# mutiann/few-shot-transformer-tts

Hardware: AMD Instinct MI355X
Metric: padded mel-frames/sec, full training step (fwd+loss+bwd+allreduce+Adam) (higher is better)
Workload: dtype bf16; 1 GPU; LJSpeech-shaped (BASELINE configs[1]) packed batch per GPU: B=14 S=114 T=582, default hparams (83.5M params), dropout on, single speaker/language; global_batch=14, seq_len=582, parallelism=dp1

## Files before the change

few-shot-transformer-tts_amd/csrc/capi_ops.hip:

```cpp
#include "engine.h"
#include "attention.h"
#include "enc_fused.h"

namespace {
inline hipStream_t S_(void* s) { return (hipStream_t)s; }
inline int rup8(int x) { return (x + 7) & ~7; }
__global__ void k_dropmask(DropCfg d, uint8_t* out, long n) {
    long i = (long)blockIdx.x * blockDim.x + threadIdx.x;
    if (i < n) out[i] = b2s_keep(d, (uint32_t)i) ? 1 : 0;
}
}

int b2s_attn_core_fwd_export(int dtype, hipStream_t st, const void* q, int ldq, const void* k, int ldk, const void* v, int ldv,
                             void* ctx, int ldc, int B, int H, int Lq, int Lk, int dh, int mask_mode, const int* klen,
                             const float* bias, long bias_sb, long bias_sq, DropCfg drop, float* S, void* P, void* Pd);
int b2s_attn_core_bwd_export(int dtype, hipStream_t st, const void* dctx, int ldc, const void* q, int ldq, const void* k, int ldk,
                             const void* v, int ldv, const void* P, const void* Pd, void* dq, int lddq, void* dk, int lddk,
                             void* dv, int lddv, int B, int H, int Lq, int Lk, int dh, DropCfg drop, float* dP, void* dS);

extern "C" int b2s_gemm(const b2s_gemm_desc* d, const void* A, const void* B, void* C, const float* bias,
                        const float* residual, const int32_t* row_len, const int32_t* conv_len, void* stream) {
    B2S_CHECK(d && A && B && C, "null argument");
    GemmArgs g;
    g.M = d->M; g.N = d->N; g.K = d->K; g.batch = d->batch > 0 ? d->batch : 1; g.batch_inner = d->batch_inner > 0 ? d->batch_inner : 1;
    g.A.p = A; g.A.ld = d->lda; g.A.bs_o = d->a_bs_o; g.A.bs_i = d->a_bs_i;
    g.B.p = B; g.B.ld = d->ldb; g.B.bs_o = d->b_bs_o; g.B.bs_i = d->b_bs_i;
    if (d->trans_a) { g.A.R = d->K; g.A.C = d->M; } else { g.A.R = d->M; g.A.C = d->K; }
    if (d->trans_b) { g.B.R = d->K; g.B.C = d->N; } else { g.B.R = d->N; g.B.C = d->K; }
    if (d->conv_cin_a > 0) {
        B2S_CHECK(!d->trans_a, "conv gather is defined on the row-major A operand");
        g.A.g_cin = d->conv_cin_a; g.A.g_T = d->conv_T; g.A.g_len = conv_len; g.A.R = d->M; g.A.C = d->K;
    }
    g.C = C; g.c_fp32 = d->c_fp32; g.ldc = d->ldc; g.cs_o = d->c_bs_o; g.cs_i = d->c_bs_i;
    g.epi.alpha = d->alpha; g.epi.bias = bias; g.epi.relu = d->relu; g.epi.accumulate = d->accumulate;
    g.epi.drop = make_drop(d->drop_p, d->seed, 7u);
    g.epi.residual = residual; g.epi.ldr = d->ldc;
    g.epi.row_len = row_len; g.epi.rows_per_batch = d->rows_per_batch > 0 ? d->rows_per_batch : 1;
    g.epi.conv_dw_cin = d->conv_dw_cin;
    return b2s_gemm_launch(g, d->dtype, d->trans_a != 0, d->trans_b != 0, S_(stream));
}
extern "C" int b2s_gemm_splitk(const b2s_gemm_desc* d, int splitk, const void* A, const void* B, float* C, float* ws, size_t ws_floats,
                               void* stream) {
    B2S_CHECK(d && A && B && C && splitk >= 1, "null argument / bad split");
    B2S_CHECK(d->c_fp32 && d->accumulate && !d->relu && d->drop_p == 0.f && d->conv_cin_a == 0, "split-K needs a linear fp32 accumulate epilogue");
    GemmArgs g;
    g.M = d->M; g.N = d->N; g.K = d->K; g.batch = d->batch > 0 ? d->batch : 1; g.batch_inner = d->batch_inner > 0 ? d->batch_inner : 1;
    g.A.p = A; g.A.ld = d->lda; g.A.bs_o = d->a_bs_o; g.A.bs_i = d->a_bs_i;
    g.B.p = B; g.B.ld = d->ldb; g.B.bs_o = d->b_bs_o; g.B.bs_i = d->b_bs_i;
    if (d->trans_a) { g.A.R = d->K; g.A.C = d->M; } else { g.A.R = d->M; g.A.C = d->K; }
    if (d->trans_b) { g.B.R = d->K; g.B.C = d->N; } else { g.B.R = d->N; g.B.C = d->K; }
    g.C = C; g.c_fp32 = 1; g.ldc = d->ldc; g.cs_o = d->c_bs_o; g.cs_i = d->c_bs_i;
    g.epi.alpha = d->alpha; g.epi.accumulate = 1; g.epi.conv_dw_cin = d->conv_dw_cin;
    g.splitk = splitk; g.ws = ws; g.ws_floats = ws ? ws_floats : 0;
// ... 151 lines not shown
```

few-shot-transformer-tts_amd/csrc/engine.hip:

```cpp
#include <algorithm>
#include <cmath>
#include <cstdarg>
#include <cstdlib>
#include "engine.h"
#include "attention.h"
#include "enc_fused.h"
#include "drop_sites.h"

thread_local char g_b2s_err[512] = "";
int b2s_fail(const char* file, int line, const char* fmt, ...) {
    char msg[400];
    va_list ap; va_start(ap, fmt); vsnprintf(msg, sizeof(msg), fmt, ap); va_end(ap);
    const char* base = strrchr(file, '/');
    snprintf(g_b2s_err, sizeof(g_b2s_err), "%s:%d: %s", base ? base + 1 : file, line, msg);
    return 1;
}

int b2s_model::id(const std::string& n) const {
    auto it = index.find(n);
    return it == index.end() ? -1 : it->second;
}

namespace {

// ... 571 lines not shown
    const int rings = m->dw_group ? cf.n_decoder_layer : 1;
    for (int i = 0; i < (rings == 1 ? 1 : 3 * rings); ++i) sc.r_dyT.push_back(a.T(M * D, esz));
    for (int i = 0; i < (rings == 1 ? 1 : 2 * rings); ++i) sc.r_dqkv.push_back(a.T(M * 3 * D, esz));
    for (int i = 0; i < rings; ++i) { sc.r_dz.push_back(a.T(M * 4 * D, esz)); sc.r_dkv.push_back(a.T(Mk * 2 * D, esz)); }
    sc.dyT = sc.r_dyT[0]; sc.dz = sc.r_dz[0]; sc.dqkv = sc.r_dqkv[0]; sc.dkv = sc.r_dkv[0];
    sc.dctx = a.T(M * D, esz); sc.dh = a.T(M * D, esz); sc.dx = a.f32(M * D);
    sc.dmelT = a.T(M * cf.num_mels, esz); sc.doutT = a.T(M * D, esz); sc.da3 = a.T(M * D, esz);
    sc.dz1 = a.T(M * cf.prenet_hidden, esz); sc.dz2 = a.T(M * cf.prenet_hidden, esz);
    sc.dstop_m = a.f32(M);
    if (m->kv_cat) sc.dkvcat = a.T(Mk * cf.n_decoder_layer * 2 * D, esz);
    sc.lnws = a.f32((long)RO_LN_WS_ROWS * 2 * D);
    for (int i = 0; i < (m->dw_group ? 3 * cf.n_decoder_layer + 2 : RO_LN_BATCH); ++i) sc.r_lnws.push_back(a.f32((long)RO_LN_WS_ROWS * 2 * D));
    if (m->kv_cat) { sc.dctx_x = a.T(M * D, esz); sc.dsum_x = a.f32((long)B * H * T); }
}

struct PostScratch { std::vector<void*> du, dy; float* stat; int stat_stride; void* col = nullptr; };
void plan_postnet(const b2s_model* m, b2s_ctx& c, Arena& a, PostScratch& ps) {
    const b2s_config& cf = m->cfg;
    const long M = (long)c.B * c.T;
    const int n = cf.n_postnet_layer, esz = m->esz;
    c.u.assign(n, nullptr); c.y.assign(n, nullptr); c.bn_mean.assign(n, nullptr); c.bn_rstd.assign(n, nullptr);
    ps.du.assign(n + 1, nullptr);
    for (int i = 0; i < n; ++i) {
        int cin = i == 0 ? cf.num_mels : cf.postnet_hidden;
        int cout = i == n - 1 ? cf.num_mels : cf.postnet_hidden;
        c.u[i] = a.T(M * cin, esz);
        c.y[i] = a.f32(M * cout);
        c.bn_mean[i] = a.f32(cout); c.bn_rstd[i] = a.f32(cout);
        ps.du[i] = a.T(M * cin, esz);
    }
    int maxc = std::max(cf.num_mels, cf.postnet_hidden);
    ps.du[n] = a.T(M * maxc, esz);
    ps.dy.assign(n, nullptr);
    for (int i = 0; i < n; ++i) ps.dy[i] = a.T(M * (i == n - 1 ? cf.num_mels : cf.postnet_hidden), esz);
    ps.stat_stride = 2 * maxc;
    ps.stat = a.f32((long)n * ps.stat_stride);
    if (m->dtype == 1) ps.col = a.T(M * 5 * maxc, esz);
}

int check_bound(const b2s_model* m) {
    B2S_CHECK(m && m->bound, "model parameters are not bound (call b2s_model_bind first)");
    return 0;
}

}

extern "C" const char* b2s_last_error(void) { return g_b2s_err; }
extern "C" int b2s_version(void) { return 100; }

extern "C" int b2s_model_create(const b2s_config* cfg, b2s_model** out) {
    B2S_CHECK(cfg && out, "null argument");
    const b2s_config& c = *cfg;
// ... 1184 lines not shown
}

extern "C" int b2s_postnet_backward(b2s_model* m, b2s_ctx* c, const float* d_out, float* d_inputs_out, int flags, void* stream) {
    B2S_TRY(check_bound(m));
    B2S_CHECK(c && c->kind == 3 && d_out && d_inputs_out, "bad postnet context");
    B2S_CHECK(c->train, "postnet backward requires a train-mode forward (batch statistics)");
    const b2s_config& cf = m->cfg;
    hipStream_t st = S_(stream);
    const int B = c->B, T = c->T, n = cf.n_postnet_layer, dt = m->dtype;
    const long M = (long)B * T;
    const float pd = cf.decoder_dropout_rate;
    Arena a; a.base = c->ws; a.cap = c->ws_bytes;
    b2s_ctx tmp; tmp.B = B; tmp.T = T;
    PostScratch ps;
    plan_postnet(m, tmp, a, ps);
    std::vector<GemmArgs> dws;
    for (int i = n - 1; i >= 0; --i) {
        const int cin = i == 0 ? cf.num_mels : cf.postnet_hidden, cout = i == n - 1 ? cf.num_mels : cf.postnet_hidden;
        const std::string q = "postnet.batchnorm_layers." + std::to_string(i) + ".";
        DropCfg d = make_drop(pd, c->seed, drop_op(DS_POST_CONV, i));
        const void* dout = i == n - 1 ? (const void*)d_out : ps.du[i + 1];
        void* dy = ps.dy[i];
        B2S_TRY(ro_bn_bwd(dt, dout, i == n - 1 ? 1 : 0, c->y[i], c->bn_mean[i], c->bn_rstd[i], m->P(q + "weight"), m->P(q + "bias"),
                          i < n - 1 ? 1 : 0, m->G(q + "weight"), m->G(q + "bias"), dy, (int)M, cout, d, st));
        {
            GemmArgs g;
            g.A.p = dy; g.A.ld = cout; g.A.R = (int)M; g.A.C = cout;
            g.B.p = c->u[i]; g.B.ld = cin; g.B.R = (int)M; g.B.C = 5 * cin; g.B.g_cin = cin; g.B.g_T = T; g.B.g_len = c->tgt_len;
            g.M = cout; g.N = 5 * cin; g.K = (int)M;
            g.C = m->G("postnet.conv_layers." + std::to_string(i) + ".weight"); g.c_fp32 = 1; g.ldc = 5 * cin;
            g.epi.conv_dw_cin = cin; g.epi.accumulate = 1; g.splitk = pick_splitk(cout, 5 * cin, (int)M, dt);
            if (m->aux) dws.push_back(g);
            else { m->set_ws(g, st); B2S_TRY(b2s_gemm_launch(g, dt, true, true, st)); }
        }
        {
            GemmArgs g;
            g.A.p = dy; g.A.ld = cout; g.A.R = (int)M; g.A.C = 5 * cout; g.A.g_cin = cout; g.A.g_T = T; g.A.g_len = nullptr;
            g.B.p = m->conv_wb[i]; g.B.ld = 5 * cout; g.B.R = cin; g.B.C = 5 * cout;
            g.M = (int)M; g.N = cin; g.K = 5 * cout;
            g.epi.row_len = c->tgt_len; g.epi.rows_per_batch = T;
            if (i == 0) { g.C = d_inputs_out; g.c_fp32 = 1; } else { g.C = ps.du[i]; g.c_fp32 = 0; }
            g.ldc = cin;
            B2S_TRY(b2s_gemm_launch(g, dt, false, false, st));
        }
    }
    if (!dws.empty()) {
        hipEvent_t ready = m->next_event();
        B2S_HIP(hipEventRecord(ready, st));
        B2S_HIP(hipStreamWaitEvent(m->aux, ready, 0));
        for (GemmArgs& g : dws) {
            if (ps.col && g.B.g_cin % 8 == 0) {
                B2S_TRY(ro_im2col5(dt, g.B.p, g.B.g_len, g.B.g_T, g.B.g_cin, ps.col, (long)g.B.R, m->aux));
                g.B.p = ps.col; g.B.ld = 5 * g.B.g_cin; g.B.g_cin = 0; g.B.g_T = 0; g.B.g_len = nullptr;
            }
            m->set_ws(g, m->aux); B2S_TRY(b2s_gemm_launch(g, dt, true, true, m->aux));
        }
        hipEvent_t done = m->next_event();
        B2S_HIP(hipEventRecord(done, m->aux));
        m->aux_dirty = true;
        m->pending_ev = done;
    }
    if ((flags & B2S_POST_BWD_DEFER_JOIN) && m->aux) {
        B2S_TRY(flush_ln_jobs(m, st));
        m->pending_stages.push_back(0);
        return 0;
    }
    B2S_TRY(join_aux(m, st));
    B2S_TRY(hook_after_stream(m, st));
    fire_stages(m, m->pending_stages);
    m->stage_done(0);
    m->pending_ev = nullptr;
// ... 206 lines not shown
```

few-shot-transformer-tts_amd/csrc/gemm.h:

```cpp
#pragma once
#include "b2s_common.h"

struct GemmOperand {
    const void* p = nullptr;
    long bs_o = 0, bs_i = 0;
    int ld = 0;
    int R = 0, C = 0;
    int g_cin = 0, g_T = 0;
    const int* g_len = nullptr;
};

struct GemmEpilogue {
    float alpha = 1.f;
    const float* bias = nullptr;
    int relu = 0;
    const void* relu_aux = nullptr;
    int ld_aux = 0;
    float aux_scale = 1.f;
    DropCfg drop = {0, 0, 1.f};
    const int* drop_salt = nullptr;
    const float* residual = nullptr;
    int ldr = 0;
    const int* row_len = nullptr;
    int rows_per_batch = 1;
// ... 14 lines not shown
    int c_fp32 = 0;
    int ldc = 0;
    long cs_o = 0, cs_i = 0;
    GemmEpilogue epi;
    float* ws = nullptr;
    size_t ws_floats = 0;
};

int b2s_gemm_launch(const GemmArgs& g, int dtype, bool ta, bool tb, hipStream_t stream);
int b2s_gemm_glds_launch(const GemmArgs& g, bool ta, bool tb, hipStream_t stream);
int b2s_gemm_skinny_launch(const GemmArgs& g, int dtype, hipStream_t stream);
long b2s_gemm_glds256_tiles(const GemmArgs& g);
int b2s_gemm_glds256_launch(const GemmArgs& g, bool ta, bool tb, const bf16_t* zero, hipStream_t stream);
int b2s_splitk_reduce_launch(const float* ws, float* dst, int M, int N, int ldc, int splitk, int conv_dw_cin, hipStream_t stream);
#define B2S_MAX_GROUP 8
struct b2s_gemm_group { int n; int order; int tile0[B2S_MAX_GROUP + 1]; GemmArgs p[B2S_MAX_GROUP]; };
int b2s_gemm_glds256_grouped_launch(const GemmArgs* probs, int n, const bf16_t* zero, hipStream_t stream);
const bf16_t* b2s_gemm_zero_page();
int b2s_gemm_grouped_launch(const GemmArgs* probs, int n, hipStream_t stream);
```

few-shot-transformer-tts_amd/csrc/gemm.hip:

```cpp
#include <mutex>
#include "gemm.h"
#include "gemm_epi.h"

namespace {

constexpr int BM = 128, BN = 128;

constexpr int BK = 16, KSTEP = 4, VE = 4;

__device__ inline float frag_n(const float* tile, int LD, int row0, int k0, int i, int g) {
    return tile[(row0 + i) * LD + k0 + g];
}
__device__ inline float frag_t(const float* tile, int LD, int row0, int k0, int i, int g) {
    return tile[(k0 + g) * LD + row0 + i];
}
__device__ inline f32x4_t mma(float a, float b, f32x4_t c) {
    return __builtin_amdgcn_mfma_f32_16x16x4f32(a, b, c, 0, 0, 0);
}

template <typename T>
__device__ inline uint4 load_chunk(const GemmOperand& o, const T* base, int r, int c) {
    uint4 z = make_uint4(0, 0, 0, 0);
    if (o.g_cin > 0) {
        if (r >= o.R || c >= o.C) return z;
// ... 217 lines not shown
    B2S_HIP(hipEventRecord(r.a, stream));
    int rc = gemm_launch_inner(g, dtype, ta, tb, stream);
    B2S_HIP(hipEventRecord(r.b, stream));
    { std::lock_guard<std::mutex> lock(g_prof_mu); g_prof.push_back(r); }
    return rc;
}
int b2s_gemm_grouped_launch(const GemmArgs* probs, int n, hipStream_t stream) {
    if (!g_prof_on) return b2s_gemm_glds256_grouped_launch(probs, n, b2s_gemm_zero_page(), stream);
    ProfRec r;
    B2S_HIP(hipEventCreate(&r.a)); B2S_HIP(hipEventCreate(&r.b));
    r.variant = 16; r.flops = 0.0;
    for (int i = 0; i < n; ++i) r.flops += 2.0 * probs[i].M * probs[i].N * (double)probs[i].K;
    r.M = probs[0].M; r.N = probs[0].N; r.K = probs[0].K; r.batch = n; r.splitk = 1;
    B2S_HIP(hipEventRecord(r.a, stream));
    int rc = b2s_gemm_glds256_grouped_launch(probs, n, b2s_gemm_zero_page(), stream);
    B2S_HIP(hipEventRecord(r.b, stream));
    { std::lock_guard<std::mutex> lock(g_prof_mu); g_prof.push_back(r); }
    return rc;
}
static int gemm_launch_inner(const GemmArgs& g, int dtype, bool ta, bool tb, hipStream_t stream) {
    const int ve = dtype ? 8 : 4;
    B2S_CHECK(g.M > 0 && g.N > 0 && g.K > 0 && g.batch > 0 && g.batch_inner > 0, "gemm: bad shape M=%d N=%d K=%d batch=%d",
              g.M, g.N, g.K, g.batch);
    B2S_CHECK(g.A.p && g.B.p && g.C, "gemm: null pointer");
    B2S_CHECK(g.A.ld % ve == 0 && g.B.ld % ve == 0, "gemm: leading dimensions (%d, %d) must be multiples of %d", g.A.ld,
              g.B.ld, ve);
    B2S_CHECK(((uintptr_t)g.A.p % 16 == 0) && ((uintptr_t)g.B.p % 16 == 0), "gemm: operands must be 16-byte aligned");
    B2S_CHECK(g.A.bs_o % ve == 0 && g.A.bs_i % ve == 0 && g.B.bs_o % ve == 0 && g.B.bs_i % ve == 0,
              "gemm: batch strides must be multiples of %d elements", ve);
    B2S_CHECK(g.batch * g.splitk <= 65535, "gemm: batch too large");
// ... 14 lines not shown
```

few-shot-transformer-tts_amd/csrc/gemm_glds256.hip:

```cpp
#include <algorithm>
#include <vector>
#include <cstdlib>
#include <mutex>
#include <atomic>
#include "gemm.h"
#include "gemm_epi.h"

#ifndef B2S_DMA_AUX
#define B2S_DMA_AUX 0
#endif

#ifndef B2S_GROUP_M
#define B2S_GROUP_M 4
#endif
#ifndef B2S_NPROD
#define B2S_NPROD 4
#endif

namespace t256 {

constexpr int NPROD = B2S_NPROD, GROUP_M = B2S_GROUP_M;
constexpr int nprod_of(int gather, int mw = 4) { return gather == 1 ? 0 : NPROD * mw / 4; }
constexpr int nthreads_of(int gather, int mw = 4) { return 64 * (2 * mw + nprod_of(gather, mw)); }
template <int N> __device__ __forceinline__ void wait_vm() { asm volatile("s_waitcnt vmcnt(%0)" ::"n"(N) : "memory"); }
// ... 36 lines not shown
        s.r = row; s.c = (pc ^ swz_n(row)) << 3;
    } else {
        const int unit = idx >> 3, qi = idx & 7;
        const int khalf = IS_A ? (unit >> 1) : unit, chalf = IS_A ? (unit & 1) : 0;
        const int krl = qi * 4 + (lane >> 4), pc = lane & 15;
        s.r = khalf * 32 + krl; s.c = chalf * 128 + ((pc ^ swz_t(krl)) << 3);
    }
    return s;
}

__device__ inline int xcd_tile_id(int orig, int nwg) {
    const int xcd = orig & 7, q = nwg >> 3, r = nwg & 7;
    return (xcd < r ? xcd * (q + 1) : r * (q + 1) + (xcd - r) * q) + (orig >> 3);
}

template <bool TA, bool TB, int GATHER, int NB, int MW = 4>
__device__ __forceinline__ void gemm256_body(GemmArgs g, const bf16_t* zero, float* splitk_ws, int bx, int by, int bz) {
    extern __shared__ __attribute__((aligned(16))) unsigned char smem_raw[];
    static_assert(MW == 4 || (MW == 2 && !TA && GATHER == 0), "128-row tiles: plain K-contiguous A only");
    constexpr int NP = nprod_of(GATHER, MW), NC = 2 * MW;
    constexpr int BMt = MW * 64, A_B = BMt * BK * 2, STG = A_B + B_BYTES;

    const int tid = threadIdx.x, lane = tid & 63;
    const int wave = __builtin_amdgcn_readfirstlane(tid >> 6);
    const int li = lane & 15, lg = lane >> 4;
    constexpr int BN = NB * 32;
    const int wrow = (wave >> 1) * 64, wcol = (wave & 1) * (NB * 16);
    const int m0 = by * BMt, n0 = bx * BN;
    const int z = bz / g.splitk, ksplit = bz - z * g.splitk;
    const int zo = z / g.batch_inner, zi = z - zo * g.batch_inner;
    const bf16_t* Ab = reinterpret_cast<const bf16_t*>(g.A.p) + zo * g.A.bs_o + zi * g.A.bs_i;
    const bf16_t* Bb = reinterpret_cast<const bf16_t*>(g.B.p) + zo * g.B.bs_o + zi * g.B.bs_i;
// ... 34 lines not shown
    }
    const int nfull = g.K / BK;
    constexpr bool GF = GATHER == 2;
    int gt[GF ? NIA : 1], glim[GF ? NIA : 1];
    if (GF) {
        const float inv_T = __builtin_amdgcn_rcpf((float)g.A.g_T);
#pragma unroll
        for (int i = 0; i < NIA; ++i) {
            const LaneSrc s = lane_src<false, true>(ia0 + i, lane);
            const int r = min(m0 + s.r, g.A.R - 1), b = fast_div(r, g.A.g_T, inv_T);
            gt[i] = r - b * g.A.g_T;
            glim[i] = g.A.g_len ? min(g.A.g_len[b], g.A.g_T) : g.A.g_T;
        }
    }
    const int g_spt = GF ? g.A.g_cin / BK : 1;
    const bool fast_ok = GATHER != 1 && nfull > 0 && (TA ? (g.A.C >= 8 && (g.A.C & 7) == 0) : true) && (TB ? (g.B.C >= 8 && (g.B.C & 7) == 0) : true) &&
                         (TA ? (long)g.A.R * g.A.ld : (long)g.A.R * g.A.ld) < (1L << 30) && (long)g.B.R * g.B.ld < (1L << 30);
    const bool b_active0 = NP || NB == 4 || TB || wave * 2 + 0 < 12, b_active1 = NP || NB == 4 || TB || wave * 2 + 1 < 12;
    const bool six = b_active0 && b_active1;

    const int nk_all = (g.K + BK - 1) / BK;
    const int per = (nk_all + g.splitk - 1) / g.splitk;
    const int kt0 = ksplit * per;
    const int kt_end = min(nk_all, kt0 + per);
    const int nk = kt_end - kt0;
    if (nk <= 0) return;

    auto issue = [&](int kt, int slot) {
        unsigned char* sbase = smem_raw + slot * STG;
        if (fast_ok && (kt < nfull || kt >= kt_end)) {
            const long ks = min(kt, nfull - 1);
            const char* sa = reinterpret_cast<const char*>(Ab) + ks * stepA * 2;
            const char* sb = reinterpret_cast<const char*>(Bb) + ks * stepB * 2;
            if (GF) {
                const int j = fast_div((int)ks, g_spt, __builtin_amdgcn_rcpf((float)g_spt)), ci0 = ((int)ks - j * g_spt) * BK;
                sa = reinterpret_cast<const char*>(Ab) + ((long)(j - 2) * g.A.ld + ci0) * 2;
#pragma unroll
                for (int i = 0; i < NIA; ++i) {
                    const bool ok = (unsigned)(gt[i] + j - 2) < (unsigned)glim[i];
                    const char* src = ok ? sa + goffA[i] : reinterpret_cast<const char*>(zero);
                    __builtin_amdgcn_global_load_lds((gptr_t)src, (lptr_t)(sbase + (ia0 + i) * 1024), 16, 0, B2S_DMA_AUX);
                }
            } else {
#pragma unroll
// ... 142 lines not shown

template <bool TA, bool TB, int GATHER, int NB, int MW = 4>
__global__ __launch_bounds__(nthreads_of(GATHER, MW), 1) void gemm_glds256_kernel(GemmArgs g, const bf16_t* zero, float* splitk_ws, int tiles_m, int tiles_n) {
    const int wg = xcd_tile_id(blockIdx.x, gridDim.x);
    const int per_z = tiles_n * tiles_m;
    const int bz = wg / per_z, rem = wg - bz * per_z;
    int by, bx;
    if (GROUP_M > 0 && tiles_n >= 16) {
        const int gsz = GROUP_M * tiles_n, grp = rem / gsz, in = rem - grp * gsz;
        const int rows = min(GROUP_M, tiles_m - grp * GROUP_M);
        bx = in / rows; by = grp * GROUP_M + (in - bx * rows);
    } else { by = rem / tiles_n; bx = rem - by * tiles_n; }
    gemm256_body<TA, TB, GATHER, NB, MW>(g, zero, splitk_ws, bx, by, bz);
}

template <int NB>
__global__ __launch_bounds__(nthreads_of(false), 1) void gemm_glds256_grouped_kernel(b2s_gemm_group grp, const bf16_t* zero) {
    const int i = blockIdx.x, xcd = i & 7;
    int p = 0, local;
    if (grp.order == 1) {
        const int T = grp.tile0[grp.n];
        int start = 0;
        for (int x = 0; x < xcd; ++x) start += (T - x + 7) >> 3;
        const int g = start + (i >> 3);
        while (p + 1 < grp.n && g >= grp.tile0[p + 1]) ++p;
        local = g - grp.tile0[p];
    } else {
        while (p + 1 < grp.n && i >= grp.tile0[p + 1]) ++p;
        const int s0 = grp.tile0[p], cnt = grp.tile0[p + 1] - s0;
        int before = 0;
        for (int x = 0; x < xcd; ++x) {
            const int first = s0 + ((x - s0) & 7);
            before += first < s0 + cnt ? (s0 + cnt - 1 - first) / 8 + 1 : 0;
        }
        local = before + (i - (s0 + ((xcd - s0) & 7))) / 8;
    }
    const int tiles_n = (grp.p[p].N + NB * 32 - 1) / (NB * 32), tiles_m = (grp.p[p].M + BM - 1) / BM;
    const int sk = grp.p[p].splitk, t = local / sk, bz = local - t * sk;
    int by, bx;
    if (grp.order == 1 && tiles_n > 8) { bx = t / tiles_m; by = t - bx * tiles_m; }
    else { by = t / tiles_n; bx = t - by * tiles_n; }
    gemm256_body<true, true, 0, NB>(grp.p[p], zero, nullptr, bx, by, bz);
}

constexpr int PST_STG = NSTAGE * STAGE_BYTES, PST_TQ = PST_STG + 8 * 1024, PST_LDS = PST_TQ + 64;
constexpr int PST_END = 0x7fffffff;

template <int NB, int MODE>
__device__ __forceinline__ void epi_small(const EpiFast& e, const DropCfg dcfg, f32x4_t (&acc)[4][NB], unsigned stg, int mb, int nb, int lane) {
    typedef uint32_t u32x4 __attribute__((ext_vector_type(4)));
    typedef uint32_t u32x2 __attribute__((ext_vector_type(2)));
    constexpr int CH = NB * 2, TASKS = 8 * CH;
    const int li = lane & 15, lg = lane >> 4;
    const int trow = lane / CH, tch = lane - trow * CH;
    const bool tvalid = lane < TASKS;
    u32x4 qa[MODE == 2 ? 8 : 1];
// ... 410 lines not shown
            }
        }
        return end;
    };
    const long deep = makespan(true), shallow = makespan(false);
    if (deep <= shallow) makespan(true);
    int tiles = 0;
    for (int k = 0; k < n; ++k) {
        const GemmArgs& g = probs[order[k]];
        B2S_CHECK(g.batch == 1 && g.c_fp32 && g.A.g_cin == 0 && g.B.g_cin == 0, "grouped GEMM: problem %d is not a plain fp32 dW", order[k]);
        grp.p[k] = g; grp.p[k].splitk = 1;
        grp.tile0[k] = tiles;
        tiles += cdiv(g.M, t256::BM) * cdiv(g.N, 128);
    }
    grp.tile0[n] = tiles;
    constexpr size_t smem = (size_t)t256::NSTAGE * t256::STAGE_BYTES;
    static std::once_flag attr_once;
    static hipError_t attr_err = hipSuccess;
    std::call_once(attr_once, [] {
        attr_err = hipFuncSetAttribute(reinterpret_cast<const void*>(t256::gemm_glds256_grouped_kernel<4>),
                                       hipFuncAttributeMaxDynamicSharedMemorySize, (int)smem);
    });
    B2S_HIP(attr_err);
    hipLaunchKernelGGL((t256::gemm_glds256_grouped_kernel<4>), dim3(tiles), dim3(t256::nthreads_of(false)), smem, stream, grp, zero);
    B2S_LAUNCH_CHECK();
    return 0;
}

extern "C" int b2s_gemm_set_tile_policy(int policy) {
    if (policy != 0 && policy != 3 && policy != 4) return b2s_fail(__FILE__, __LINE__, "tile policy must be 0 (auto), 3 (256x96) or 4 (256x128), got %d", policy);
    t256::g_tile_policy.store(policy, std::memory_order_relaxed);
    return 0;
}

long b2s_gemm_glds256_tiles(const GemmArgs& g) { return (long)cdiv(g.M, t256::BM) * cdiv(g.N, 128) * g.batch * std::max(1, g.splitk); }

int b2s_gemm_glds256_launch(const GemmArgs& g, bool ta, bool tb, const bf16_t* zero, hipStream_t stream) {
    const bool gather = g.A.g_cin > 0 || g.B.g_cin > 0;
    if (gather) {
        if (!ta && !tb) {
            const bool aligned = g.A.g_cin > 0 && g.B.g_cin == 0 && g.A.g_cin % t256::BK == 0 && g.K % t256::BK == 0 && g.splitk == 1 &&
                                 (long)g.A.R * g.A.ld < (1L << 29) && (long)g.B.R * g.B.ld < (1L << 30) && g.A.g_T > 0;
            if (aligned) return t256::launch256_t<false, false, 2>(g, zero, stream);
// ... 11 lines not shown
```

few-shot-transformer-tts_amd/csrc/rowops.h:

```cpp
#pragma once
#include "b2s_common.h"

int ro_embed_prep_fwd(const long* ids, const int* lens, const float* embed, const float* pe, const float* pe_scale,
                      float* x, int B, int S, int D, DropCfg drop, hipStream_t st);
int ro_embed_prep_bwd(const float* dx, const long* ids, const int* lens, const float* pe, float* d_embed,
                      float* d_pe_scale, int B, int S, int D, DropCfg drop, hipStream_t st, int dx_bf16 = 0);

int ro_layernorm_fwd(int dtype, const float* x, const float* gamma, const float* beta, void* y, int ldy, float* y32,
                     int ldy32, float* mean, float* rstd, int M, int D, float eps, const int* row_len,
                     int rows_per_batch, hipStream_t st);
int ro_layernorm_bwd(int dtype, const void* dy, int dy_fp32, int lddy, const float* x, const float* gamma,
                     const float* mean, const float* rstd, float* dx, int accumulate, float* dgamma, float* dbeta,
                     int M, int D, const int* row_len, int rows_per_batch, hipStream_t st, float* ws = nullptr,
                     void* dy2 = nullptr, DropCfg drop2 = DropCfg{0, 0, 1.f}, int* defer_nblk = nullptr, int dx_bf16 = 0);
constexpr int RO_LN_WS_ROWS = 768;
struct LnReduceJob { const float* ws; int nblk, D; float* dgamma; float* dbeta; };
constexpr int RO_LN_BATCH = 8;
struct LnReduceBatch { int n; LnReduceJob j[RO_LN_BATCH]; };
int ro_ln_param_reduce_batch(const LnReduceBatch& b, hipStream_t st);

int ro_softmax_fwd(int dtype, const float* S, void* P, void* Pd, int B, int H, int Lq, int Lk, int ldp, float scale,
                   int mask_mode, const int* klen, const float* bias, long bias_sb, long bias_sq, DropCfg drop,
                   hipStream_t st);
int ro_softmax_bwd(int dtype, const void* P, const float* dPraw, void* dS, int B, int H, int Lq, int Lk, int ldp,
// ... 52 lines not shown
                hipStream_t st);

struct MtChunk {
    float* a; float* b; float* c; float* d; bf16_t* s; int n; int pad;
    bf16_t* s2; int cin, cout; long off;
};
int ro_mt_sumsq(const MtChunk* chunks, int nchunks, float* out, float scale, hipStream_t st);
int ro_mt_param_wire(const MtChunk* chunks, int nchunks, float* wire, const float* gbase, bool scatter, hipStream_t st);
int ro_mt_cast(const MtChunk* chunks, int nchunks, hipStream_t st);
int ro_mt_zero(const MtChunk* chunks, int nchunks, hipStream_t st);
int ro_mt_axpy(const MtChunk* chunks, int nchunks, float alpha, const float* gscale, hipStream_t st);
struct AdamHyper { float lr, bc1, sbc2; };
int ro_mt_adam(const MtChunk* chunks, int nchunks, AdamHyper hp, float beta1, float beta2, float eps, float l2,
               float grad_scale, float* sumsq_part, hipStream_t st, const void* wire = nullptr, const float* gbase = nullptr,
               int max_wg = 0);
int ro_im2col5(int dtype, const void* x, const int* lens, int T, int cin, void* out, long M, hipStream_t st);
int ro_sum_scaled(const float* part, int n, float scale, float* out, hipStream_t st, float* zero = nullptr, int nzero = 0);

int ro_conv_w_relayout(int dtype, const float* w, void* wf, void* wb, int Cout, int Cin, hipStream_t st);
int ro_add(const float* a, const float* b, float* out, long n, hipStream_t st);
int ro_add3(const float* a, const float* b, const float* c, float* out, long n, hipStream_t st);
```

few-shot-transformer-tts_amd/csrc/rowops.hip:

```cpp
#include <algorithm>
#include <cstdlib>
#include "rowops.h"

namespace {

#define RO_DISPATCH(dtype, CALL) do { if (dtype) { typedef bf16_t TY; CALL; } else { typedef float TY; CALL; } } while (0)

__device__ inline float4 ld4(const float* p) { return *reinterpret_cast<const float4*>(p); }
__device__ inline void st4(float* p, float4 v) { *reinterpret_cast<float4*>(p) = v; }
__device__ inline float4 ld4(const bf16_t* p) {
    uint2 u = *reinterpret_cast<const uint2*>(p);
    return make_float4(bf2f(u.x & 0xffff), bf2f(u.x >> 16), bf2f(u.y & 0xffff), bf2f(u.y >> 16));
}
__device__ inline void st4(bf16_t* p, float4 v) {
    uint2 u;
    u.x = f2bf2(v.x, v.y);
    u.y = f2bf2(v.z, v.w);
    *reinterpret_cast<uint2*>(p) = u;
}
__device__ inline float4 drop4(float4 v, const DropCfg& d, uint32_t idx) {
    if (!d.thresh) return v;
    v.x = b2s_keep(d, idx) ? v.x * d.scale : 0.f;
    v.y = b2s_keep(d, idx + 1) ? v.y * d.scale : 0.f;
    v.z = b2s_keep(d, idx + 2) ? v.z * d.scale : 0.f;
// ... 1410 lines not shown
    constexpr bool v1 = false;
    const int grid = max_wg > 0 ? std::min(max_wg, nchunks) : nchunks;
    if (nchunks > 0 && wire)
        hipLaunchKernelGGL(k_mt_adam2<true>, dim3(grid), dim3(256), 0, st, chunks, nchunks, hp, beta1, beta2, eps, l2, grad_scale, sumsq_part, (const bf16_t*)wire, gbase);
    else if (nchunks > 0 && v1)
        hipLaunchKernelGGL(k_mt_adam, dim3(nchunks), dim3(256), 0, st, chunks, hp, beta1, beta2, eps, l2, grad_scale, sumsq_part);
    else if (nchunks > 0)
        hipLaunchKernelGGL(k_mt_adam2<false>, dim3(grid), dim3(256), 0, st, chunks, nchunks, hp, beta1, beta2, eps, l2, grad_scale, sumsq_part, (const bf16_t*)nullptr,
                           (const float*)nullptr);
    B2S_LAUNCH_CHECK(); return 0;
}
int ro_sum_scaled(const float* part, int n, float scale, float* out, hipStream_t st, float* zero, int nzero) {
    hipLaunchKernelGGL(k_sum_scaled, dim3(1), dim3(1024), 0, st, part, n, scale, out, zero, nzero);
    B2S_LAUNCH_CHECK(); return 0;
}
__global__ __launch_bounds__(256) void k_im2col5(const uint4* __restrict__ x, const int* __restrict__ lens, int T, int c8, uint4* __restrict__ out, long M) {
    const long total = M * 5 * c8;
    for (long i = (long)blockIdx.x * 256 + threadIdx.x; i < total; i += (long)gridDim.x * 256) {
        const long m = i / (5 * c8);
        const int rem = (int)(i - m * 5 * c8), j = rem / c8, c = rem - j * c8;
        const int b = (int)(m / T), t = (int)(m - (long)b * T), ts = t + j - 2;
        const int lim = lens ? min(lens[b], T) : T;
        const bool ok = (unsigned)ts < (unsigned)lim;
        const uint4 v = x[(ok ? m + j - 2 : m) * c8 + c];
        out[i] = ok ? v : make_uint4(0, 0, 0, 0);
    }
}
int ro_im2col5(int dtype, const void* x, const int* lens, int T, int cin, void* out, long M, hipStream_t st) {
    B2S_CHECK(dtype == 1 && cin % 8 == 0 && T > 0, "im2col: bf16 rows of a multiple of 8 channels only");
    const long total = M * 5 * (cin / 8);
    hipLaunchKernelGGL(k_im2col5, dim3((int)std::min<long>(cdiv(total, 256), 4096)), dim3(256), 0, st, (const uint4*)x, lens, T, cin / 8, (uint4*)out, M);
    B2S_LAUNCH_CHECK(); return 0;
}
int ro_conv_w_relayout(int dtype, const float* w, void* wf, void* wb, int Cout, int Cin, hipStream_t st) {
    RO_DISPATCH(dtype, hipLaunchKernelGGL((k_conv_w_relayout<TY>), dim3(ew_grid((long)Cout * Cin * 5)), dim3(256), 0, st, w,
                                          (TY*)wf, (TY*)wb, Cout, Cin));
    B2S_LAUNCH_CHECK(); return 0;
}
int ro_add3(const float* a, const float* b, const float* c, float* out, long n, hipStream_t st) {
    hipLaunchKernelGGL(k_add3, dim3(ew_grid(n)), dim3(256), 0, st, a, b, c, out, n);
    B2S_LAUNCH_CHECK(); return 0;
}
int ro_add(const float* a, const float* b, float* out, long n, hipStream_t st) {
    hipLaunchKernelGGL(k_add, dim3(ew_grid(n)), dim3(256), 0, st, a, b, out, n);
    B2S_LAUNCH_CHECK(); return 0;
}
__global__ __launch_bounds__(256) void k_mt_cast(const MtChunk* __restrict__ ch) {
    const MtChunk c = ch[blockIdx.x];
// ... 69 lines not shown
```

Measured before the change: 1.235 million mel-frames/s.

## Compute postnet conv weight gradients from shifted token-row segments without im2col

The postnet conv weight gradient used to be built by materializing a 5x im2col buffer for each layer and then running a GEMM over it. Now the grouped glds256 GEMM kernel treats each of the 5 taps as its own output tile column. For each batch it walks K over valid time segments, shifting the input rows by the tap offset and skipping padding rows. All postnet layers are launched as one grouped kernel, removing the im2col kernel, its scratch buffer and the extra memory traffic. The risk is more tiles, shorter K segments with partial-tile edge handling, and a dependence on the producer-wave path constraints.

```diff
diff --git a/few-shot-transformer-tts_amd/csrc/capi_ops.hip b/few-shot-transformer-tts_amd/csrc/capi_ops.hip
--- a/few-shot-transformer-tts_amd/csrc/capi_ops.hip
+++ b/few-shot-transformer-tts_amd/csrc/capi_ops.hip
@@ -37,6 +37,16 @@
     g.epi.residual = residual; g.epi.ldr = d->ldc;
     g.epi.row_len = row_len; g.epi.rows_per_batch = d->rows_per_batch > 0 ? d->rows_per_batch : 1;
     g.epi.conv_dw_cin = d->conv_dw_cin;
+    if (d->conv_dw_cin > 0 && d->conv_T > 0 && d->conv_cin_a == 0) {
+        B2S_CHECK(d->dtype == 1 && d->trans_a && d->trans_b && g.batch == 1 && d->c_fp32 && d->alpha == 1.f && !bias && !residual && !row_len && !d->relu &&
+                  d->drop_p == 0.f, "conv dW on token rows: bf16 TN form, fp32 output, linear epilogue");
+        B2S_CHECK(d->N == 5 * d->conv_dw_cin && d->K % d->conv_T == 0, "conv dW on token rows: N = %d must be 5 cin (cin = %d), K = %d a multiple of T = %d",
+                  d->N, d->conv_dw_cin, d->K, d->conv_T);
+        GemmArgs w;
+        w.A.p = A; w.A.ld = d->lda; w.B.p = B; w.B.ld = d->ldb; w.M = d->M; w.N = d->conv_dw_cin; w.K = d->K;
+        w.C = C; w.c_fp32 = 1; w.ldc = d->ldc; w.epi.accumulate = d->accumulate;
+        return b2s_gemm_conv_dw_launch(&w, 1, conv_len, d->K / d->conv_T, d->conv_T, S_(stream));
+    }
     return b2s_gemm_launch(g, d->dtype, d->trans_a != 0, d->trans_b != 0, S_(stream));
 }
 extern "C" int b2s_gemm_splitk(const b2s_gemm_desc* d, int splitk, const void* A, const void* B, float* C, float* ws, size_t ws_floats,
diff --git a/few-shot-transformer-tts_amd/csrc/engine.hip b/few-shot-transformer-tts_amd/csrc/engine.hip
--- a/few-shot-transformer-tts_amd/csrc/engine.hip
+++ b/few-shot-transformer-tts_amd/csrc/engine.hip
@@ -609,7 +609,7 @@
     if (m->kv_cat) { sc.dctx_x = a.T(M * D, esz); sc.dsum_x = a.f32((long)B * H * T); }
 }
 
-struct PostScratch { std::vector<void*> du, dy; float* stat; int stat_stride; void* col = nullptr; };
+struct PostScratch { std::vector<void*> du, dy; float* stat; int stat_stride; };
 void plan_postnet(const b2s_model* m, b2s_ctx& c, Arena& a, PostScratch& ps) {
     const b2s_config& cf = m->cfg;
     const long M = (long)c.B * c.T;
@@ -630,7 +630,6 @@
     for (int i = 0; i < n; ++i) ps.dy[i] = a.T(M * (i == n - 1 ? cf.num_mels : cf.postnet_hidden), esz);
     ps.stat_stride = 2 * maxc;
     ps.stat = a.f32((long)n * ps.stat_stride);
-    if (m->dtype == 1) ps.col = a.T(M * 5 * maxc, esz);
 }
 
 int check_bound(const b2s_model* m) {
@@ -1845,7 +1844,7 @@
     b2s_ctx tmp; tmp.B = B; tmp.T = T;
     PostScratch ps;
     plan_postnet(m, tmp, a, ps);
-    std::vector<GemmArgs> dws;
+    std::vector<GemmArgs> dws, segs;
     for (int i = n - 1; i >= 0; --i) {
         const int cin = i == 0 ? cf.num_mels : cf.postnet_hidden, cout = i == n - 1 ? cf.num_mels : cf.postnet_hidden;
         const std::string q = "postnet.batchnorm_layers." + std::to_string(i) + ".";
@@ -1854,7 +1853,14 @@
         void* dy = ps.dy[i];
         B2S_TRY(ro_bn_bwd(dt, dout, i == n - 1 ? 1 : 0, c->y[i], c->bn_mean[i], c->bn_rstd[i], m->P(q + "weight"), m->P(q + "bias"),
                           i < n - 1 ? 1 : 0, m->G(q + "weight"), m->G(q + "bias"), dy, (int)M, cout, d, st));
-        {
+        if (dt == 1 && cin % 8 == 0 && cout % 8 == 0) {
+            GemmArgs g;
+            g.A.p = dy; g.A.ld = cout; g.B.p = c->u[i]; g.B.ld = cin;
+            g.M = cout; g.N = cin; g.K = (int)M;
+            g.C = m->G("postnet.conv_layers." + std::to_string(i) + ".weight"); g.c_fp32 = 1; g.ldc = 5 * cin;
+            g.epi.accumulate = 1;
+            segs.push_back(g);
+        } else {
             GemmArgs g;
             g.A.p = dy; g.A.ld = cout; g.A.R = (int)M; g.A.C = cout;
             g.B.p = c->u[i]; g.B.ld = cin; g.B.R = (int)M; g.B.C = 5 * cin; g.B.g_cin = cin; g.B.g_T = T; g.B.g_len = c->tgt_len;
@@ -1875,17 +1881,18 @@
             B2S_TRY(b2s_gemm_launch(g, dt, false, false, st));
         }
     }
-    if (!dws.empty()) {
+    auto launch_segs = [&](hipStream_t s) -> int {
+        for (size_t i = 0; i < segs.size(); i += B2S_MAX_GROUP)
+            B2S_TRY(b2s_gemm_conv_dw_launch(segs.data() + i, (int)std::min<size_t>(B2S_MAX_GROUP, segs.size() - i), c->tgt_len, B, T, s));
+        return 0;
+    };
+    if (!m->aux) B2S_TRY(launch_segs(st));
+    else if (!dws.empty() || !segs.empty()) {
         hipEvent_t ready = m->next_event();
         B2S_HIP(hipEventRecord(ready, st));
         B2S_HIP(hipStreamWaitEvent(m->aux, ready, 0));
-        for (GemmArgs& g : dws) {
-            if (ps.col && g.B.g_cin % 8 == 0) {
-                B2S_TRY(ro_im2col5(dt, g.B.p, g.B.g_len, g.B.g_T, g.B.g_cin, ps.col, (long)g.B.R, m->aux));
-                g.B.p = ps.col; g.B.ld = 5 * g.B.g_cin; g.B.g_cin = 0; g.B.g_T = 0; g.B.g_len = nullptr;
-            }
-            m->set_ws(g, m->aux); B2S_TRY(b2s_gemm_launch(g, dt, true, true, m->aux));
-        }
+        for (GemmArgs& g : dws) { m->set_ws(g, m->aux); B2S_TRY(b2s_gemm_launch(g, dt, true, true, m->aux)); }
+        B2S_TRY(launch_segs(m->aux));
         hipEvent_t done = m->next_event();
         B2S_HIP(hipEventRecord(done, m->aux));
         m->aux_dirty = true;
diff --git a/few-shot-transformer-tts_amd/csrc/gemm.h b/few-shot-transformer-tts_amd/csrc/gemm.h
--- a/few-shot-transformer-tts_amd/csrc/gemm.h
+++ b/few-shot-transformer-tts_amd/csrc/gemm.h
@@ -52,7 +52,10 @@
 int b2s_gemm_glds256_launch(const GemmArgs& g, bool ta, bool tb, const bf16_t* zero, hipStream_t stream);
 int b2s_splitk_reduce_launch(const float* ws, float* dst, int M, int N, int ldc, int splitk, int conv_dw_cin, hipStream_t stream);
 #define B2S_MAX_GROUP 8
-struct b2s_gemm_group { int n; int order; int tile0[B2S_MAX_GROUP + 1]; GemmArgs p[B2S_MAX_GROUP]; };
+struct b2s_gemm_group { int n; int order; int tile0[B2S_MAX_GROUP + 1]; GemmArgs p[B2S_MAX_GROUP];
+                        const int* seg_len; int seg_n, seg_T; };
 int b2s_gemm_glds256_grouped_launch(const GemmArgs* probs, int n, const bf16_t* zero, hipStream_t stream);
+int b2s_gemm_glds256_conv_dw_launch(const GemmArgs* probs, int n, const int* len, int B, int T, const bf16_t* zero, hipStream_t stream);
+int b2s_gemm_conv_dw_launch(const GemmArgs* probs, int n, const int* len, int B, int T, hipStream_t stream);
 const bf16_t* b2s_gemm_zero_page();
 int b2s_gemm_grouped_launch(const GemmArgs* probs, int n, hipStream_t stream);
diff --git a/few-shot-transformer-tts_amd/csrc/gemm.hip b/few-shot-transformer-tts_amd/csrc/gemm.hip
--- a/few-shot-transformer-tts_amd/csrc/gemm.hip
+++ b/few-shot-transformer-tts_amd/csrc/gemm.hip
@@ -255,6 +255,21 @@
     r.M = probs[0].M; r.N = probs[0].N; r.K = probs[0].K; r.batch = n; r.splitk = 1;
     B2S_HIP(hipEventRecord(r.a, stream));
     int rc = b2s_gemm_glds256_grouped_launch(probs, n, b2s_gemm_zero_page(), stream);
+    B2S_HIP(hipEventRecord(r.b, stream));
+    { std::lock_guard<std::mutex> lock(g_prof_mu); g_prof.push_back(r); }
+    return rc;
+}
+int b2s_gemm_conv_dw_launch(const GemmArgs* probs, int n, const int* len, int B, int T, hipStream_t stream) {
+    const bf16_t* zero = b2s_gemm_zero_page();
+    if (!zero) return 1;
+    if (!g_prof_on) return b2s_gemm_glds256_conv_dw_launch(probs, n, len, B, T, zero, stream);
+    ProfRec r;
+    B2S_HIP(hipEventCreate(&r.a)); B2S_HIP(hipEventCreate(&r.b));
+    r.variant = 16; r.flops = 0.0;
+    for (int i = 0; i < n; ++i) r.flops += 2.0 * probs[i].M * 5.0 * probs[i].N * (double)B * T;
+    r.M = probs[0].M; r.N = 5 * probs[0].N; r.K = B * T; r.batch = n; r.splitk = 1;
+    B2S_HIP(hipEventRecord(r.a, stream));
+    int rc = b2s_gemm_glds256_conv_dw_launch(probs, n, len, B, T, zero, stream);
     B2S_HIP(hipEventRecord(r.b, stream));
     { std::lock_guard<std::mutex> lock(g_prof_mu); g_prof.push_back(r); }
     return rc;
diff --git a/few-shot-transformer-tts_amd/csrc/gemm_glds256.hip b/few-shot-transformer-tts_amd/csrc/gemm_glds256.hip
--- a/few-shot-transformer-tts_amd/csrc/gemm_glds256.hip
+++ b/few-shot-transformer-tts_amd/csrc/gemm_glds256.hip
@@ -74,8 +74,16 @@
     return (xcd < r ? xcd * (q + 1) : r * (q + 1) + (xcd - r) * q) + (orig >> 3);
 }
 
-template <bool TA, bool TB, int GATHER, int NB, int MW = 4>
-__device__ __forceinline__ void gemm256_body(GemmArgs g, const bf16_t* zero, float* splitk_ws, int bx, int by, int bz) {
+struct ConvSeg { const int* len; int n, T, shift; };
+__device__ __forceinline__ void conv_seg(const ConvSeg& sg, int b, int& row, int& klen) {
+    const int len = sg.len ? min(max(sg.len[b], 0), sg.T) : sg.T;
+    const int t0 = max(0, -sg.shift), t1 = min(sg.T, len - sg.shift);
+    row = b * sg.T + t0; klen = max(t1 - t0, 0);
+}
+
+template <bool TA, bool TB, int GATHER, int NB, int MW = 4, bool SEG = false>
+__device__ __forceinline__ void gemm256_body(GemmArgs g, const bf16_t* zero, float* splitk_ws, int bx, int by, int bz, const ConvSeg sg = ConvSeg{nullptr, 0, 0, 0}) {
+    static_assert(!SEG || (TA && TB && GATHER == 0 && MW == 4 && NPROD > 0), "K segments: the producer-wave TN form only");
     extern __shared__ __attribute__((aligned(16))) unsigned char smem_raw[];
     static_assert(MW == 4 || (MW == 2 && !TA && GATHER == 0), "128-row tiles: plain K-contiguous A only");
     constexpr int NP = nprod_of(GATHER, MW), NC = 2 * MW;
@@ -140,20 +148,56 @@
         }
     }
     const int g_spt = GF ? g.A.g_cin / BK : 1;
-    const bool fast_ok = GATHER != 1 && nfull > 0 && (TA ? (g.A.C >= 8 && (g.A.C & 7) == 0) : true) && (TB ? (g.B.C >= 8 && (g.B.C & 7) == 0) : true) &&
+    const bool fast_ok = GATHER != 1 && (SEG || nfull > 0) && (TA ? (g.A.C >= 8 && (g.A.C & 7) == 0) : true) && (TB ? (g.B.C >= 8 && (g.B.C & 7) == 0) : true) &&
                          (TA ? (long)g.A.R * g.A.ld : (long)g.A.R * g.A.ld) < (1L << 30) && (long)g.B.R * g.B.ld < (1L << 30);
     const bool b_active0 = NP || NB == 4 || TB || wave * 2 + 0 < 12, b_active1 = NP || NB == 4 || TB || wave * 2 + 1 < 12;
     const bool six = b_active0 && b_active1;
 
-    const int nk_all = (g.K + BK - 1) / BK;
+    int nk_all = (g.K + BK - 1) / BK;
+    if (SEG) {
+        nk_all = 0;
+        for (int b = 0; b < sg.n; ++b) { int row, klen; conv_seg(sg, b, row, klen); nk_all += (klen + BK - 1) / BK; }
+    }
+    int sg_b = -1, sg_first = 0, sg_steps = 0, sg_klen = 0, sg_row = 0;
     const int per = (nk_all + g.splitk - 1) / g.splitk;
     const int kt0 = ksplit * per;
     const int kt_end = min(nk_all, kt0 + per);
     const int nk = kt_end - kt0;
-    if (nk <= 0) return;
+    if (!SEG && nk <= 0) return;
 
     auto issue = [&](int kt, int slot) {
         unsigned char* sbase = smem_raw + slot * STG;
+        if (SEG) {
+            while (kt >= sg_first + sg_steps && sg_b + 1 < sg.n) {
+                sg_first += sg_steps; ++sg_b;
+                conv_seg(sg, sg_b, sg_row, sg_klen);
+                sg_steps = (sg_klen + BK - 1) / BK;
+            }
+            const int ks = kt - sg_first, left = sg_klen - ks * BK;
+            const long ra = sg_row + ks * BK, rb = ra + sg.shift;
+            if (fast_ok && left >= BK) {
+                const char* sa = reinterpret_cast<const char*>(Ab) + ra * g.A.ld * 2;
+                const char* sb = reinterpret_cast<const char*>(Bb) + rb * g.B.ld * 2;
+#pragma unroll
+                for (int i = 0; i < NIA; ++i)
+                    __builtin_amdgcn_global_load_lds((gptr_t)(sa + goffA[i]), (lptr_t)(sbase + (ia0 + i) * 1024), 16, 0, B2S_DMA_AUX);
+#pragma unroll
+                for (int i = 0; i < NIB; ++i)
+                    __builtin_amdgcn_global_load_lds((gptr_t)(sb + goffB[i]), (lptr_t)(sbase + A_B + (ib0 + i) * 1024), 16, 0, B2S_DMA_AUX);
+                return;
+            }
+#pragma unroll
+            for (int i = 0; i < NIA; ++i) {
+                const bf16_t* sa = (ka[i] >= 0 && ka[i] < left) ? pa[i] + ra * g.A.ld : zero;
+                __builtin_amdgcn_global_load_lds((gptr_t)sa, (lptr_t)(sbase + (ia0 + i) * 1024), 16, 0, B2S_DMA_AUX);
+            }
+#pragma unroll
+            for (int i = 0; i < NIB; ++i) {
+                const bf16_t* sb = (kb_[i] >= 0 && kb_[i] < left) ? pb[i] + rb * g.B.ld : zero;
+                __builtin_amdgcn_global_load_lds((gptr_t)sb, (lptr_t)(sbase + A_B + (ib0 + i) * 1024), 16, 0, B2S_DMA_AUX);
+            }
+            return;
+        }
         if (fast_ok && (kt < nfull || kt >= kt_end)) {
             const long ks = min(kt, nfull - 1);
             const char* sa = reinterpret_cast<const char*>(Ab) + ks * stepA * 2;
@@ -326,7 +370,7 @@
     gemm256_body<TA, TB, GATHER, NB, MW>(g, zero, splitk_ws, bx, by, bz);
 }
 
-template <int NB>
+template <int NB, bool SEG = false>
 __global__ __launch_bounds__(nthreads_of(false), 1) void gemm_glds256_grouped_kernel(b2s_gemm_group grp, const bf16_t* zero) {
     const int i = blockIdx.x, xcd = i & 7;
     int p = 0, local;
@@ -347,11 +391,20 @@
         }
         local = before + (i - (s0 + ((xcd - s0) & 7))) / 8;
     }
-    const int tiles_n = (grp.p[p].N + NB * 32 - 1) / (NB * 32), tiles_m = (grp.p[p].M + BM - 1) / BM;
+    const int tiles_tap = (grp.p[p].N + NB * 32 - 1) / (NB * 32);
+    const int tiles_n = SEG ? 5 * tiles_tap : tiles_tap, tiles_m = (grp.p[p].M + BM - 1) / BM;
     const int sk = grp.p[p].splitk, t = local / sk, bz = local - t * sk;
     int by, bx;
     if (grp.order == 1 && tiles_n > 8) { bx = t / tiles_m; by = t - bx * tiles_m; }
     else { by = t / tiles_n; bx = t - by * tiles_n; }
+    if constexpr (SEG) {
+        GemmArgs g = grp.p[p];
+        const int j = bx / tiles_tap;
+        g.C = reinterpret_cast<float*>(g.C) + j;
+        const ConvSeg sg = {grp.seg_len, grp.seg_n, grp.seg_T, j - 2};
+        gemm256_body<true, true, 0, NB, 4, true>(g, zero, nullptr, bx - j * tiles_tap, by, 0, sg);
+        return;
+    }
     gemm256_body<true, true, 0, NB>(grp.p[p], zero, nullptr, bx, by, bz);
 }
 
@@ -792,6 +845,7 @@
         tiles += cdiv(g.M, t256::BM) * cdiv(g.N, 128);
     }
     grp.tile0[n] = tiles;
+    grp.seg_len = nullptr; grp.seg_n = 0; grp.seg_T = 0;
     constexpr size_t smem = (size_t)t256::NSTAGE * t256::STAGE_BYTES;
     static std::once_flag attr_once;
     static hipError_t attr_err = hipSuccess;
@@ -805,6 +859,42 @@
     return 0;
 }
 
+int b2s_gemm_glds256_conv_dw_launch(const GemmArgs* probs, int n, const int* len, int B, int T, const bf16_t* zero, hipStream_t stream) {
+    B2S_CHECK(n >= 1 && n <= B2S_MAX_GROUP && B > 0 && T > 0 && (long)B * T < (1L << 30), "conv dW: %d layers (max %d), B = %d, T = %d", n, B2S_MAX_GROUP, B, T);
+    b2s_gemm_group grp;
+    grp.n = n; grp.order = 1;
+    grp.seg_len = len; grp.seg_n = B; grp.seg_T = T;
+    int tiles = 0;
+    for (int k = 0; k < n; ++k) {
+        GemmArgs g = probs[k];
+        B2S_CHECK(g.batch == 1 && g.c_fp32 && g.A.p && g.B.p && g.C && g.A.g_cin == 0 && g.B.g_cin == 0, "conv dW: layer %d is not a plain fp32 dW", k);
+        B2S_CHECK(g.M > 0 && g.N > 0 && g.M % 8 == 0 && g.N % 8 == 0 && g.A.ld % 8 == 0 && g.B.ld % 8 == 0 && g.A.ld >= g.M && g.B.ld >= g.N && g.ldc >= 5 * g.N,
+                  "conv dW: layer %d: cout = %d, cin = %d and the leading dimensions (%d, %d) must be multiples of 8, ldc = %d >= 5 cin", k, g.M, g.N,
+                  g.A.ld, g.B.ld, g.ldc);
+        B2S_CHECK(((uintptr_t)g.A.p % 16 == 0) && ((uintptr_t)g.B.p % 16 == 0), "conv dW: operands must be 16-byte aligned");
+        B2S_CHECK(!g.epi.bias && !g.epi.relu && !g.epi.relu_aux && !g.epi.residual && !g.epi.drop.thresh && !g.epi.row_len && !g.epi.colstat && !g.epi.kv_k,
+                  "conv dW: linear epilogue only");
+        g.A.R = g.B.R = g.K = B * T; g.A.C = g.M; g.B.C = g.N;
+        g.splitk = 1; g.ws = nullptr; g.ws_floats = 0; g.cs_o = g.cs_i = 0; g.A.bs_o = g.A.bs_i = g.B.bs_o = g.B.bs_i = 0;
+        g.epi.conv_dw_cin = g.N;
+        grp.p[k] = g;
+        grp.tile0[k] = tiles;
+        tiles += cdiv(g.M, t256::BM) * 5 * cdiv(g.N, 128);
+    }
+    grp.tile0[n] = tiles;
+    constexpr size_t smem = (size_t)t256::NSTAGE * t256::STAGE_BYTES;
+    static std::once_flag attr_once;
+    static hipError_t attr_err = hipSuccess;
+    std::call_once(attr_once, [] {
+        attr_err = hipFuncSetAttribute(reinterpret_cast<const void*>(t256::gemm_glds256_grouped_kernel<4, true>),
+                                       hipFuncAttributeMaxDynamicSharedMemorySize, (int)smem);
+    });
+    B2S_HIP(attr_err);
+    hipLaunchKernelGGL((t256::gemm_glds256_grouped_kernel<4, true>), dim3(tiles), dim3(t256::nthreads_of(false)), smem, stream, grp, zero);
+    B2S_LAUNCH_CHECK();
+    return 0;
+}
+
 extern "C" int b2s_gemm_set_tile_policy(int policy) {
     if (policy != 0 && policy != 3 && policy != 4) return b2s_fail(__FILE__, __LINE__, "tile policy must be 0 (auto), 3 (256x96) or 4 (256x128), got %d", policy);
     t256::g_tile_policy.store(policy, std::memory_order_relaxed);
diff --git a/few-shot-transformer-tts_amd/csrc/rowops.h b/few-shot-transformer-tts_amd/csrc/rowops.h
--- a/few-shot-transformer-tts_amd/csrc/rowops.h
+++ b/few-shot-transformer-tts_amd/csrc/rowops.h
@@ -90,7 +90,6 @@
 int ro_mt_adam(const MtChunk* chunks, int nchunks, AdamHyper hp, float beta1, float beta2, float eps, float l2,
                float grad_scale, float* sumsq_part, hipStream_t st, const void* wire = nullptr, const float* gbase = nullptr,
                int max_wg = 0);
-int ro_im2col5(int dtype, const void* x, const int* lens, int T, int cin, void* out, long M, hipStream_t st);
 int ro_sum_scaled(const float* part, int n, float scale, float* out, hipStream_t st, float* zero = nullptr, int nzero = 0);
 
 int ro_conv_w_relayout(int dtype, const float* w, void* wf, void* wb, int Cout, int Cin, hipStream_t st);
diff --git a/few-shot-transformer-tts_amd/csrc/rowops.hip b/few-shot-transformer-tts_amd/csrc/rowops.hip
--- a/few-shot-transformer-tts_amd/csrc/rowops.hip
+++ b/few-shot-transformer-tts_amd/csrc/rowops.hip
@@ -1448,24 +1448,6 @@
     hipLaunchKernelGGL(k_sum_scaled, dim3(1), dim3(1024), 0, st, part, n, scale, out, zero, nzero);
     B2S_LAUNCH_CHECK(); return 0;
 }
-__global__ __launch_bounds__(256) void k_im2col5(const uint4* __restrict__ x, const int* __restrict__ lens, int T, int c8, uint4* __restrict__ out, long M) {
-    const long total = M * 5 * c8;
-    for (long i = (long)blockIdx.x * 256 + threadIdx.x; i < total; i += (long)gridDim.x * 256) {
-        const long m = i / (5 * c8);
-        const int rem = (int)(i - m * 5 * c8), j = rem / c8, c = rem - j * c8;
-        const int b = (int)(m / T), t = (int)(m - (long)b * T), ts = t + j - 2;
-        const int lim = lens ? min(lens[b], T) : T;
-        const bool ok = (unsigned)ts < (unsigned)lim;
-        const uint4 v = x[(ok ? m + j - 2 : m) * c8 + c];
-        out[i] = ok ? v : make_uint4(0, 0, 0, 0);
-    }
-}
-int ro_im2col5(int dtype, const void* x, const int* lens, int T, int cin, void* out, long M, hipStream_t st) {
-    B2S_CHECK(dtype == 1 && cin % 8 == 0 && T > 0, "im2col: bf16 rows of a multiple of 8 channels only");
-    const long total = M * 5 * (cin / 8);
-    hipLaunchKernelGGL(k_im2col5, dim3((int)std::min<long>(cdiv(total, 256), 4096)), dim3(256), 0, st, (const uint4*)x, lens, T, cin / 8, (uint4*)out, M);
-    B2S_LAUNCH_CHECK(); return 0;
-}
 int ro_conv_w_relayout(int dtype, const float* w, void* wf, void* wb, int Cout, int Cin, hipStream_t st) {
     RO_DISPATCH(dtype, hipLaunchKernelGGL((k_conv_w_relayout<TY>), dim3(ew_grid((long)Cout * Cin * 5)), dim3(256), 0, st, w,
                                           (TY*)wf, (TY*)wb, Cout, Cin));
```

Measured after the change: 1.252 million mel-frames/s (median of 6 runs). 1.3% higher.
